# sharwarimarathe/GossipProtocol

Hardware: AMD Instinct MI355X
Metric: node-updates/sec (whole node) + achieved HBM GB/s %, imp3D push-sum 1e9 nodes (higher is better)
Workload: dtype f64; 1 GPU; push-sum rounds, Imp3D lattice, n=1000000000 (P=1000000000), steady state (all nodes active), seed 1; num_nodes=1000000000, population=1000000000, topology=Imp3D, algorithm=push-sum, parallelism=slab1, transport=none (one GPU), launcher=single process, activation_preroll_rounds=72

## Files before the change

gossipprotocol_amd/csrc/gp_host.hpp:

```cpp
#pragma once
#include <algorithm>
#include <array>
#include <chrono>
#include <cmath>
#include <cerrno>
#include <cstdarg>
#include <cstdio>
#include <cstdlib>
#include <cstring>
#include <optional>
#include <string>
#include <thread>
#include <vector>

#include <fcntl.h>
#include <sys/stat.h>
#include <unistd.h>

#include <rccl/rccl.h>

#include "../../include/gossip_hip.h"
#include "gp_internal.hpp"
#include "gp_full.hpp"
#include "gp_fullbin.hpp"

#include "gp_xchg.hpp"

using namespace gp;
#pragma GCC visibility push(hidden)

extern thread_local std::string g_err;
void set_err(const char* fmt, ...);
int check_device(int device);

#define HIP_TRY(expr)                                                                   \
    do {                                                                                \
        hipError_t e_ = (expr);                                                         \
        if (e_ != hipSuccess) {                                                         \
            set_err("%s failed: %s (%s:%d)", #expr, hipGetErrorString(e_), __FILE__, __LINE__); \
            return GP_EHIP;                                                             \
        }                                                                               \
    } while (0)

#define NCCL_TRY(expr)                                                                  \
    do {                                                                                \
        ncclResult_t r_ = (expr);                                                       \
        if (r_ != ncclSuccess) {                                                        \
            set_err("%s failed: %s (%s:%d)", #expr, ncclGetErrorString(r_), __FILE__, __LINE__); \
            return GP_ENCCL;                                                            \
        }                                                                               \
    } while (0)

constexpr int64_t BATCH = 1024;
static_assert(BATCH <= HIST, "alert ring must cover a batch");

struct ExpOverrides {
    KernelOverrides kernel;
    std::optional<uint32_t> fb_cap1, fb_cap2;
    std::optional<bool> fb_fused;
    std::optional<bool> rq8;
    std::optional<uint32_t> halo_cap;
    std::optional<uint32_t> xcap;
    std::optional<bool> no_pack;
    std::optional<uint32_t> ind4_wide;
    std::optional<bool> force_rccl;
    bool check_close = false;
};
ExpOverrides read_overrides();

struct Xfer { bool send; int peer; uint8_t* ptr; size_t bytes; };

struct Slab {
    DevState S{};
    int rank = 0;
    uint32_t hi = 0;
    uint32_t* pos = nullptr;
    uint8_t* xdst = nullptr;
    uint8_t* xsend = nullptr;
    uint8_t* xrecv = nullptr;
    uint32_t nedges = 0;
    XLayout xl;
    unsigned int* overflow = nullptr;
    bool lists = false;
    uint32_t nt = 0;
    uint32_t tb[XMAXH + 1] = {};
    uint32_t* gw = nullptr;
    uint16_t* xdr = nullptr;
    uint8_t* lwt = nullptr;
    uint32_t* xcnt = nullptr;
    uint8_t* xown = nullptr;
    bool bits = false;
    uint32_t* rbits_in = nullptr;
    uint32_t* tgt = nullptr;
    BitsLayout bl;
    double2* hsend[2] = {nullptr, nullptr};
    double2* hrecv[2] = {nullptr, nullptr};
    std::vector<Xfer> xhalo[2];
    std::vector<std::vector<Xfer>> xplan[2];
};

#pragma GCC visibility pop
struct gp_sim {
    gp_config cfg{};
    int device = 0;
    hipStream_t stream = nullptr;
    ExpOverrides exp;
    KernelPlan kplan;
    int grid = 1;
    int cus = 1;
    int64_t P = 0, T = 0, g = 0;
    int mode = MODE_SINGLE;
    int world = 1, rank = 0;
    std::vector<uint32_t> bounds;
    uint32_t halo = 0;
    std::vector<Slab> slab;
    ncclComm_t comm = nullptr;
    int64_t rounds_done = 0;
// ... 68 lines not shown
```

gossipprotocol_amd/csrc/gp_internal.hpp:

```cpp
#pragma once

#include <hip/hip_runtime.h>
#include <stdint.h>

#include <algorithm>
#include <cmath>
#include <vector>

#include "gp_block_plan.hpp"
#pragma GCC visibility push(hidden)
#include "gp_plan.hpp"
#include "gp_kernel_plan.hpp"
#pragma GCC visibility pop
#include "gp_device.hpp"

namespace gp {

constexpr int HIST = 4096;
constexpr uint32_t INJ_CHUNK = 65536;

constexpr int vmcnt_enc(int n) { return 0x0F70 | (n & 15) | ((n >> 4) << 14); }

template <typename T>
__device__ __forceinline__ T ld_const(const T* p) {
// ... 97 lines not shown
}

struct XHdr {
    unsigned long long mask;
    uint32_t base;
    uint32_t pad;
};
static_assert(sizeof(XHdr) == 16, "header words move as 16-byte loads");

struct DevState {
    Geom G;
    int topo, alg;
    uint32_t k0, k1;
    uint32_t seed_node;
    Ctl* ctl;
    double2* sw[2];
    uint8_t* nb[2];
    int32_t* c;
    uint32_t* rq[2];
    uint32_t rq8;
    uint32_t* rtg;
    uint32_t* sbits;
    uint64_t* rbits[2];
    uint32_t rbits_words;
    uint32_t* rnd;
    uint32_t* in_off;
    uint32_t* in_src;
    uint32_t* in_srcd;
    uint8_t* ind4;
    uint32_t* live_bits;
    uint32_t* chunk_live;
    uint32_t nchunks;
    int32_t* inc;
    uint32_t fb_s1, fb_nb1, fb_nb2, fb_cap1, fb_cap2;
    uint32_t fb_fused;
    uint32_t *fb_cnt1, *fb_cnt2;
    uint32_t *fb_hdr1, *fb_hdr2;
    double2 *fb_pay1, *fb_pay2;
    uint32_t lo, nloc, base;
    uint32_t ext_lo, ext_hi;
    uint32_t* rtag;
    double2* rmsg;
    uint32_t* rk;
    const XHdr* xhdr[2];
    const double2* xvals[2];
    uint32_t xnv;
    int kernel;
    uint32_t col_xsegs;
    uint32_t tile_walk;
    uint32_t tile_wx;
    uint32_t tile_stage_cap;
#ifdef GP_EXPERIMENTS
    uint32_t tile_no_full;
#endif
    uint32_t fuse_finalize;
    BlockPlan bplan;
    void* bface;
    void* bscratch;
    uint32_t tile_wide;
    uint32_t nedges;
    uint32_t* tq;
    uint32_t* wtiles;
    uint32_t rregions;
    uint32_t woff[RREG_MAX][9];
};
constexpr int TQ_STRIDE = 64;
hipError_t launch_round_tile_region(const DevState& S, uint32_t round, uint32_t h, int grid, hipStream_t st);

constexpr int TILE = 1024;
static_assert(XTILE == TILE, "the lists' tiles (gp_plan.hpp) are the tile kernels' tiles");

struct RoundArgs {
    const double2* swc;
    double2* swn;
    const uint8_t* nbc;
    uint8_t* nbn;
    const uint64_t* rbc;
    uint64_t* rbn;
    const uint32_t* in_off;
    const uint32_t* in_src;
    const uint32_t* in_srcd;
    const uint8_t* ind4;
    const uint32_t* rtag;
    const double2* rmsg;
    const uint32_t* rk;
    const XHdr* xhdr;
    const double2* xvals;
    uint32_t xnv;
    int32_t* c;
    Ctl* ctl;
    Geom G;
    uint32_t k0, k1, seed_node, ntiles;
    uint32_t lo, nloc, ext_lo, ext_hi;
    uint32_t walk;
    uint32_t wx;
    uint32_t stage_cap;
#ifdef GP_EXPERIMENTS
    uint32_t no_full;
#endif
    uint32_t fuse;
    const uint32_t* wt;
    uint32_t wo[9];
    uint32_t* tq;
    uint32_t* tq_next;
};

size_t block_face_bytes(const BlockPlan& p);
hipError_t block_kernel_setup(const BlockPlan& p);
bool block_plan_resident(const BlockPlan& p, int cus);
constexpr int BLOCK_EPOCH = 64;
constexpr size_t BLOCK_SCRATCH_BYTES = 4 * (144 + 12 * BLOCK_EPOCH);
hipError_t launch_round_block(const struct DevState& S, const BlockPlan& p, uint32_t r0, uint32_t nrounds, void* face,
                              void* scratch, hipStream_t st);

struct WaveArgs {
    const uint8_t* nbc;
    uint8_t* nbn;
    int32_t* c;
    uint32_t* rq_cur;
    uint32_t* rq_next;
    uint32_t rq8;
    const uint32_t* rnd;
    const uint32_t* rtg;
    uint32_t* sbits;
    Ctl* ctl;
    Geom G;
    uint32_t k0, k1, seed_node;
    uint32_t lo, nloc, base;
    uint32_t x_lo, x_hi, zsegs, yblocks, xs_len, nitems;
};

WaveArgs make_wave_args(const DevState& S, uint32_t round);

hipError_t launch_round_col(const WaveArgs& a, int topo, int alg, uint32_t round, int grid, hipStream_t st);
int col_blocks_per_cu(int topo, int alg);
hipError_t launch_col_seed_init(const DevState& S, hipStream_t st);

uint32_t rbits_words_for(uint32_t lo, uint32_t nloc);
RoundArgs make_round_args(const DevState& S, uint32_t round);
hipError_t launch_round_tile(const DevState& S, uint32_t round, int grid, hipStream_t st);
hipError_t launch_rbits_init(const DevState& S, int grid, hipStream_t st);
uint32_t ind4_bytes_for(uint32_t lo, uint32_t nloc);
hipError_t launch_pack_ind4(const DevState& S, uint32_t wide_at, int grid, hipStream_t st);
hipError_t launch_pack_src_deg(const uint32_t* src, uint32_t* out, uint32_t n, const Geom& G, int grid,
                               hipStream_t st);

hipError_t launch_ps_tile(const DevState& S, const RoundArgs& a, uint32_t round, int grid, hipStream_t st);
int ps_tile_resident_blocks(int topo, bool remote, int device);
hipError_t launch_gossip_tile(const DevState& S, const RoundArgs& a, uint32_t round, int grid, hipStream_t st);

namespace wide {
// ... 24 lines not shown
```

gossipprotocol_amd/csrc/gp_ps_tile.hip:

```cpp
#include <type_traits>

#include "gp_tile.hpp"

namespace gp {
#ifdef GP_TILE_WIDE
namespace wide {
#endif

constexpr int PRIO = 1;

namespace {

template <bool REMOTE>
struct PsSlots {
    static constexpr bool SNDPF = !REMOTE;
    static constexpr int SLOTS = SNDPF ? TILE + TILE / 8 : TILE + TILE / 8 + TILE / 16;
    static constexpr int FU = (SLOTS + TPB - 1) / TPB;
};

template <bool REMOTE>
struct TileLdsP {
    static constexpr int SLOTS = PsSlots<REMOTE>::SLOTS, SLOT_FU = PsSlots<REMOTE>::FU;
    uint32_t rows[W_ROWS + DMA_SLACK];
    uint32_t xm[W_PLANE + DMA_SLACK];
// ... 171 lines not shown
                    uint32_t hb[FU];
#pragma unroll
                    for (int m = 0; m < FU; ++m) {
                        const bool cand = pick[m] && isrc[m] - a.lo >= a.nloc;
                        const XHdr* hp = a.xhdr + (cand ? rkv[m] >> 6 : 0u);
                        hm[m] = *reinterpret_cast<const uint2*>(&hp->mask);
                        hb[m] = hp->base;
                    }
#pragma unroll
                    for (int m = 0; m < FU; ++m) asm volatile("" : "+v"(hm[m].x), "+v"(hm[m].y), "+v"(hb[m])::"memory");
#pragma unroll
                    for (int m = 0; m < FU; ++m) {
                        ridx[m] = 0u;
                        if (pick[m] && isrc[m] - a.lo >= a.nloc) {
                            const unsigned long long mk = ((unsigned long long)hm[m].y << 32) | hm[m].x;
                            const uint32_t bit = rkv[m] & 63u;
                            sent[m] = (mk >> bit) & 1ull;
                            ridx[m] = min(hb[m] + (uint32_t)__popcll(mk & ((1ull << bit) - 1ull)), a.xnv - 1u);
                        }
                    }
                }
                __builtin_amdgcn_s_setprio(PRIO);
#pragma unroll
                for (int m = 0; m < FU; ++m) {
                    const unsigned long long bal = __ballot(sent[m]);
                    if (lane == 0) L.bits[m * (TPB / 64) + wv] = bal;
                    if (sent[m]) {
                        const double2* src;
                        if constexpr (REMOTE) {
                            uint32_t xi = ridx[m];
                            asm volatile("" : "+v"(xi));
                            src = isrc[m] - a.lo >= a.nloc ? a.xvals + xi : swc + isrc[m];
                        } else {
                            src = swc + isrc[m];
                        }
                        __builtin_amdgcn_global_load_lds((gvoid_t*)src, (lvoid_t*)(L.msg + (m * TPB + wv * 64)), 16,
                                                         0, DMA_ONCE);
                    }
                }
                if (threadIdx.x == 0) {
                    unsigned long long z = 0ull;
                    asm volatile("" : "+v"(z));
                    L.bits[FU * (TPB / 64)] = z;
                }
            }
        }
        double2 own[NPT];
        const uint32_t b_rows = dma_stage_bytes(L.rows, a.nbc, (int64_t)j0 - H, (int64_t)j1 + H, a.ext_lo, a.ext_hi);
        uint32_t b_xm = 0, b_xp = 0;
        if (TOPO != LINE) {
            b_xm = dma_stage_bytes(L.xm, a.nbc, (int64_t)j0 - G.g2, (int64_t)j1 - G.g2, a.ext_lo, a.ext_hi);
            b_xp = dma_stage_bytes(L.xp, a.nbc, (int64_t)j0 + G.g2, (int64_t)j1 + G.g2, a.ext_lo, a.ext_hi);
        }
        if (lane < 2u * NPT) {
            uint32_t zl = lane;
            asm volatile("" : "+v"(zl));
            int64_t jn = (int64_t)T + (int64_t)((zl >> 1) * TPB + wv * 64u) + ((zl & 1u) ? 64 : -1);
            if (jn < (int64_t)a.ext_lo) jn = a.ext_lo;
            if (jn > (int64_t)a.ext_hi) jn = a.ext_hi;
            __builtin_amdgcn_global_load_lds((gvoid_t*)(swc + jn), (lvoid_t*)&L.zb[wv][0][0], 16, 0, 0);
        }
        if (TOPO == IMP3D) {
            const uint8_t* ip = a.ind4 + T / 2;
            asm volatile("" : "+s"(ip));
            dma_copy<DMA_ONCE>(L.ind, reinterpret_cast<const char*>(ip), TILE / 2);
        }
        if (dyn && threadIdx.x == 0) L.qn[it & 1] = claim;
        __builtin_amdgcn_s_setprio(0);
        __syncthreads();
        uint32_t cinc = 0;
        bool wide = false;
        if (TOPO == IMP3D) {
            const uint2 w2 = reinterpret_cast<const uint2*>(L.ind)[lane];
            auto nsum = [](uint32_t w) { return (((w & 0x0F0F0F0Fu) + ((w >> 4) & 0x0F0F0F0Fu)) * 0x01010101u) >> 24; };
            auto has15 = [](uint32_t w) { return (w & (w >> 1) & (w >> 2) & (w >> 3) & 0x11111111u) != 0u; };
            uint32_t incl = nsum(w2.x) + nsum(w2.y);
            wide = __ballot(has15(w2.x) || has15(w2.y)) != 0ull;
#pragma unroll
            for (int o = 1; o < 64; o <<= 1) {
                const uint32_t t = __shfl_up(incl, o, 64);
                if (lane >= (uint32_t)o) incl += t;
            }
            const uint32_t ex = __shfl_up(incl, 1, 64);
            cinc = lane == 0 ? 0u : ex;
        }
        uint32_t t_next = tw.t + tw.step;
        if (dyn) {
            t_next = __builtin_amdgcn_readfirstlane(L.qn[it & 1]);
            ++it;
            if (TOPO == IMP3D) {
                TileWalk nw = tw;
                nw.t = t_next;
                uint32_t nti;
                pf_tile = 0xFFFFFFFFu;
                if (nw.t < nw.end && nw.tile(nti)) {
                    const uint32_t nT = (a.lo / TILE + nti) * TILE;
                    pf_lo = ld_const(a.in_off + max(a.lo, nT));
                    pf_hi = ld_const(a.in_off + min(a.lo + a.nloc, nT + TILE));
                    pf_tile = nti;
                }
            }
        }

        bool full = j0 == T && j1 == T + TILE && (TOPO != IMP3D || (staged && !wide));
#ifdef GP_EXPERIMENTS
        if (a.no_full) full = false;
#endif
        auto tile_body = [&](auto full_c) {
        constexpr bool FULL = decltype(full_c)::value;
        uint32_t tid = threadIdx.x;
        asm volatile("" : "+v"(tid));
        const uint32_t lane = tid & 63u, wv = tid >> 6;
        uint32_t pend[(NPT + 1) / 2];
#pragma unroll
        for (int k = 0; k < (NPT + 1) / 2; ++k) pend[k] = 0u;
        {
            const uint32_t wbase = __builtin_amdgcn_readfirstlane(tid & ~63u);
            uint32_t wcx = 0, wcy = 0, wcz = 0;
            if (TOPO != LINE) {
                const uint32_t jw = T + wbase;
                wcx = fastdiv(jw, G.div_g2);
                const uint32_t rem = jw - wcx * G.g2;
                wcy = fastdiv(rem, G.div_g);
                wcz = rem - wcy * G.g;
            }
            constexpr uint32_t NDG = TOPO == LINE ? 0u : 4u;
            constexpr int NG = 1;
#pragma unroll
            for (int k0 = 0; k0 < NPT; k0 += NG) {
                __builtin_amdgcn_s_setprio(PRIO);
                uint32_t epre[NG], edeg[NG];
#pragma unroll
                for (int h = 0; h < NG; ++h) {
                    epre[h] = edeg[h] = 0u;
                    if (TOPO == IMP3D) {
                        const int k = k0 + h;
                        const uint32_t jl = k * TPB + tid;
                        const uint32_t d = (lds_byte(L.ind, jl >> 1) >> ((jl & 1u) * 4u)) & 15u;
                        uint32_t ex = mbcnt64(__ballot(d & 1u)) + 2u * mbcnt64(__ballot(d & 2u));
                        if (__ballot(d >= 4u)) ex += 4u * mbcnt64(__ballot(d & 4u)) + 8u * mbcnt64(__ballot(d & 8u));
                        const int wvu = __builtin_amdgcn_readfirstlane((int)wv);
                        epre[h] = (uint32_t)__builtin_amdgcn_readlane((int)cinc, 16 * k + 4 * wvu) + ex;
                        edeg[h] = d;
                    }
                }
                uint32_t gst[NG];
                double2 m[NG][NDG > 0 ? NDG : 1];
#pragma unroll
                for (int h = 0; h < NG; ++h) {
                    const int k = k0 + h;
                    const uint32_t j = T + k * TPB + tid;
                    if (TOPO != LINE && k > 0) {
                        wcz += TPB;
                        if (wcz >= G.g) {
                            const uint32_t q = fastdiv(wcz, G.div_g);
                            wcz -= q * G.g;
                            wcy += q;
                            if (wcy >= G.g) {
                                const uint32_t q2 = fastdiv(wcy, G.div_g);
                                wcy -= q2 * G.g;
                                wcx += q2;
                            }
                        }
                    }
                    const uint32_t jr = j - b_rows;
                    const uint32_t gbv = lds_byte(L.rows, jr);
                    uint32_t mask;
                    if (TOPO == LINE) {
                        mask = present_mask<TOPO>(j, G);
                    } else {
                        const uint32_t gm = G.g - 1u;
                        const bool interior = wcz >= 1u && wcz + 64u < gm && wcy >= 1u && wcy < gm && wcx >= 1u && wcx < gm;
                        mask = interior ? 63u : present_mask<TOPO>(j, G);
                    }
                    uint32_t from = 0;
                    if (TOPO == LINE) {
                        from |= ((mask & 1u) && (lds_byte(L.rows, (mask & 1u) ? jr - 1 : jr) & DIR_MASK) == 1u) ? 1u : 0u;
                        from |= ((mask & 2u) && (lds_byte(L.rows, (mask & 2u) ? jr + 1 : jr) & DIR_MASK) == 0u) ? 2u : 0u;
                    } else {
                        const uint32_t bxm = lds_byte(L.xm, (mask & 1u) ? j - G.g2 - b_xm : 0u);
                        const uint32_t bxp = lds_byte(L.xp, (mask & 2u) ? j + G.g2 - b_xp : 0u);
                        const uint32_t byp = lds_byte(L.rows, (mask & 4u) ? jr + G.g : jr);
                        const uint32_t bym = lds_byte(L.rows, (mask & 8u) ? jr - G.g : jr);
                        uint32_t bzp, bzm;
                        if constexpr (FULL) {
                            const uint32_t be = lds_byte(L.rows, lane == 63u ? jr + 1u : max(jr, 1u) - 1u);
                            bzp = (uint32_t)__builtin_amdgcn_mov_dpp((int)gbv, 0x130, 0xF, 0xF, true);
                            bzm = (uint32_t)__builtin_amdgcn_mov_dpp((int)gbv, 0x138, 0xF, 0xF, true);
                            if (lane == 63u) bzp = be;
                            if (lane == 0u) bzm = be;
                        } else {
                            bzp = lds_byte(L.rows, (mask & 16u) ? jr + 1 : jr);
                            bzm = lds_byte(L.rows, (mask & 32u) ? jr - 1 : jr);
                        }
                        from =((bxm & DIR_MASK) == 1u ? 1u : 0u) | ((bxp & DIR_MASK) == 0u ? 2u : 0u) |
                               ((byp & DIR_MASK) == 3u ? 4u : 0u) | ((bym & DIR_MASK) == 2u ? 8u : 0u) |
                               ((bzp & DIR_MASK) == 5u ? 16u : 0u) | ((bzm & DIR_MASK) == 4u ? 32u : 0u);
                        from &= mask;
                    }
                    if (!FULL && !(j >= j0 && j < j1)) from = 0u;
                    gst[h] = gbv | (mask << 8) | (from << 14) | (edeg[h] << 20);
                    own[k] = swc[FULL ? j : min(max(j, j0), j1 - 1u)];
#pragma unroll
                    for (uint32_t d = 0; d < NDG; ++d)
                        m[h][d] = ld_sw(swc + ((from >> d) & 1u ? nbr<TOPO>(j, d, G) : a.ext_hi));
                }
                __builtin_amdgcn_s_setprio(0);
#pragma unroll
                for (int h = 0; h < NG; ++h) {
                    const int k = k0 + h;
                    const uint32_t jl = k * TPB + tid;
                    const uint32_t j = T + jl;
                    const bool valid = FULL || (j >= j0 && j < j1);
                    uint32_t pwin = 0u, pqb = 0u;
                    if (TOPO == IMP3D && (FULL || (staged && !wide))) {
                        const uint32_t* bw = reinterpret_cast<const uint32_t*>(L.bits);
                        pqb = epre[h];
                        const uint32_t nd = gst[h] >> 20;
                        pwin = __builtin_amdgcn_alignbit(bw[(pqb >> 5) + 1], bw[pqb >> 5], pqb & 31u) & ((1u << nd) - 1u);
                    }
                    double2 zP = make_double2(0.0, 0.0), zM = zP;
                    {
                        constexpr uint32_t dP = TOPO == LINE ? 1u : 4u, dM = TOPO == LINE ? 0u : 5u;
                        const uint32_t from = (gst[h] >> 14) & 63u;
                        zP = dpp_double2<0x130>(own[k]);
                        zM = dpp_double2<0x138>(own[k]);
                        if (lane == 63u) zP = L.zb[wv][k][1];
                        if (lane == 0u) zM = L.zb[wv][k][0];
                        if (!((from >> dP) & 1u)) zP = make_double2(0.0, 0.0);
                        else if (!FULL && lane != 63u && j + 1u >= j1) zP = ld_sw(swc + j + 1);
                        if (!((from >> dM) & 1u)) zM = make_double2(0.0, 0.0);
                        else if (!FULL && lane != 0u && j <= j0) zM = ld_sw(swc + j - 1);
                    }
                    __builtin_amdgcn_s_waitcnt(vmcnt_enc(0));
                    if (valid) {
                        const uint32_t b = gst[h] & 0xFFu, mask = (gst[h] >> 8) & 63u, from = (gst[h] >> 14) & 63u;
                        const uint32_t deg = popc6(mask) + (TOPO == IMP3D ? 1u : 0u);
                        bool active = (b & B_ACTIVE) != 0;
                        const double2 sv = own[k];

                        const bool halve = active && deg > 0;
                        const double hf = halve ? 0.5 : 1.0;
                        double acc_s = sv.x * hf;
                        double acc_w = sv.y * hf;
                        auto fold = [&](const double2 mi) {
                            acc_s = __builtin_fma(mi.x, 0.5, acc_s);
                            acc_w = __builtin_fma(mi.y, 0.5, acc_w);
                        };
                        tiny |= (sv.y < 0x1p-1020) | (sv.x != 0.0 && sv.x < 0x1p-1020);
                        bool recv = from != 0;
                        if (TOPO == LINE) {
                            fold(zM);
                            fold(zP);
                        } else {
#pragma unroll
                            for (uint32_t d = 0; d < NDG; ++d) fold(m[h][d]);
                            fold(zP);
                            fold(zM);
                        }
                        if (TOPO == IMP3D) {
                            uint32_t e_b = e_lo + epre[h], e_e = e_b + (gst[h] >> 20);
                            if (!FULL && wide) {
                                e_b = a.in_off[j];
                                e_e = a.in_off[j + 1];
                            }
                            if (FULL || (staged && !wide)) {
                                uint32_t win = pwin;
                                while (win) {
                                    const uint32_t q = pqb + (uint32_t)__builtin_ctz(win);
                                    win &= win - 1u;
                                    fold(L.msg[q]);
                                    recv = true;
                                }
                            } else if (staged) {
                                const uint32_t* bw = reinterpret_cast<const uint32_t*>(L.bits);
                                const uint32_t qe = e_e - e_lo;
                                for (uint32_t q0 = e_b - e_lo; q0 < qe; q0 += 32u) {
                                    uint32_t win = __builtin_amdgcn_alignbit(bw[(q0 >> 5) + 1], bw[q0 >> 5], q0 & 31u);
                                    if (qe - q0 < 32u) win &= (1u << (qe - q0)) - 1u;
                                    while (win) {
                                        const uint32_t q = q0 + (uint32_t)__builtin_ctz(win);
                                        win &= win - 1u;
                                        fold(L.msg[q]);
                                        recv = true;
                                    }
                                }
                            } else {
                                for (uint32_t e = e_b; e < e_e; ++e) {
                                    const uint32_t i = in_src[e];
                                    bool sent;
                                    double2 mi = make_double2(0.0, 0.0);
                                    const bool rem = REMOTE && i - a.lo >= a.nloc;
                                    uint32_t xi = 0;
                                    if (rem) {
                                        const uint32_t k = a.rk[e];
                                        const XHdr h = a.xhdr[k >> 6];
                                        sent = (h.mask >> (k & 63u)) & 1ull;
                                        xi = min(h.base + (uint32_t)__popcll(h.mask & ((1ull << (k & 63u)) - 1ull)),
                                                 a.xnv - 1u);
                                    } else if (all_active) {
                                        const uint32_t di = popc6(present_mask<IMP3D>(i, G)) + 1u;
                                        sent = uniform(a.k0, a.k1, S_PUSHSUM, i, r, di) == di - 1u;
                                    } else {
                                        sent = (rbc[(i >> 6) - (a.lo >> 6)] >> (i & 63)) & 1ull;
                                    }
                                    if (sent) mi = rem ? a.xvals[xi] : ld_sw(swc + i);
                                    if (sent) {
                                        fold(mi);
                                        recv = true;
                                    }
                                }
                            }
                        }
                        uint32_t flags = b & (B_ACTIVE | B_CONV | (3u << CNT_SHIFT));
                        if (recv) {
                            if (!(b & B_CONV)) {
                                uint32_t cnt3 = (b >> CNT_SHIFT) & 3u;
                                cnt3 = ratio_moved(sv.x, sv.y, acc_s, acc_w) ? 0u : cnt3 + 1u;
                                flags = (flags & ~(3u << CNT_SHIFT)) | (cnt3 << CNT_SHIFT);
                                if (cnt3 == 3) {
                                    flags |= B_CONV;
                                    ++alerts;
                                }
                            }
                            if (!active) {
                                ++newly;
                                flags |= B_ACTIVE;
                                active = true;
                            }
                        }
                        pend[k >> 1] |= (mask | (active && deg > 0 ? 64u : 0u) | ((flags >> 3) << 7)) << (16 * (k & 1));
                        st_stream(swn + j, make_double2(acc_s, acc_w));
                    }
                }
                if (SNDPF && TOPO == IMP3D && k0 == 0) {
                    snd_tile = 0xFFFFFFFFu;
                    if (pf_tile != 0xFFFFFFFFu && pf_hi - pf_lo <= cap) {
                        snd_off = dma_stage_words(snd, srcp, pf_lo, pf_hi);
                        snd_tile = pf_tile;
                    }
                }
            }
        }
        {
            uint32_t node[NPT], x[NPT], y[NPT];
#pragma unroll
            for (int k = 0; k < NPT; ++k) node[k] = T + k * TPB + tid;
            philox2_batch<NPT>(node, r + 1, S_PUSHSUM, a.k0, a.k1, x, y);
#pragma unroll
            for (int k = 0; k < NPT; ++k) {
                const uint32_t jl = k * TPB + tid;
                const bool valid = FULL || (node[k] >= j0 && node[k] < j1);
                const uint32_t pk = pend[k >> 1] >> (16 * (k & 1));
                const uint32_t mask = pk & 63u;
                uint32_t dir = DIR_NONE;
                if (pk & 64u) dir = slot_to_dir_fast(mask, uniform_from(x[k], y[k], popc6(mask) + (TOPO == IMP3D ? 1u : 0u)));
                if (valid) reinterpret_cast<uint8_t*>(L.out)[jl] = (uint8_t)((((pk >> 7) & 15u) << 3) | dir);
                if (TOPO == IMP3D) {
                    const unsigned long long bits = __ballot(valid && dir == DIR_RANDOM);
                    if (lane == 0) {
                        const int64_t wi = (int64_t)((T + k * TPB + (tid & ~63u)) >> 6) - (int64_t)(a.lo >> 6);
                        if (wi >= 0) a.rbn[wi] = bits;
                    }
                }
            }
        }
        __syncthreads();
        for (uint32_t w = tid; w < (uint32_t)(TILE / 4); w += TPB) {
            const uint32_t jw = T + w * 4;
            if (FULL || (jw >= j0 && jw + 4 <= j1)) {
                st_stream(reinterpret_cast<uint32_t*>(a.nbn + T) + w, L.out[w]);
            } else {
                for (uint32_t b = 0; b < 4; ++b)
                    if (jw + b >= j0 && jw + b < j1) a.nbn[jw + b] = reinterpret_cast<const uint8_t*>(L.out)[w * 4 + b];
            }
        }
        };
        if (full) tile_body(std::true_type{});
        else tile_body(std::false_type{});
        tw.t = t_next;
    }
        if (!dyn || ++victim >= 8u) break;
        const uint32_t c = (blockIdx.x + victim) & 7u;
        tw.qc = a.tq + c * TQ_STRIDE;
        tw.wl = a.wt + a.wo[c];
        tw.end = a.wo[c + 1] - a.wo[c];
        if (threadIdx.x == 0) L.qn[it & 1] = atomicAdd(tw.qc, 1u);
        __syncthreads();
        tw.t = __builtin_amdgcn_readfirstlane(L.qn[it & 1]);
        ++it;
    }
}

__device__ __forceinline__ void block_counts(uint32_t (*red)[TPB / 64], uint32_t& x, uint32_t& y) {
    uint32_t tid = threadIdx.x;
    asm volatile("" : "+v"(tid));
    const uint32_t lane = tid & 63u, wv = tid >> 6;
#pragma unroll
    for (int o = 32; o > 0; o >>= 1) {
        x += __shfl_xor(x, o, 64);
        y += __shfl_xor(y, o, 64);
    }
    if (lane == 0) {
        red[0][wv] = x;
        red[1][wv] = y;
    }
    __syncthreads();
    if (threadIdx.x == 0) {
        x = 0;
        y = 0;
        for (int w = 0; w < TPB / 64; ++w) {
            x += red[0][w];
            y += red[1][w];
        }
    }
}

__device__ __forceinline__ void add_round_counts(Ctl* ctl, uint32_t x, uint32_t y) {
    unsigned long long d = 0;
    if (x) d += __hip_atomic_fetch_add(&ctl->round_alerts, (unsigned long long)x, __ATOMIC_RELAXED,
                                       __HIP_MEMORY_SCOPE_AGENT);
    if (y) d += __hip_atomic_fetch_add(&ctl->round_active, (unsigned long long)y, __ATOMIC_RELAXED,
                                       __HIP_MEMORY_SCOPE_AGENT);
    asm volatile("" ::"v"(d));
    __builtin_amdgcn_s_waitcnt(0);
}

template <int TOPO, bool REMOTE>
__global__ __launch_bounds__(TPB, GP_MINB) void k_ps_tile(RoundArgs a, uint32_t r) {
    __shared__ TileLdsP<REMOTE> L;
    __shared__ uint32_t snd[PsSlots<REMOTE>::SNDPF ? PsSlots<REMOTE>::SLOTS + DMA_SLACK : 1];
    Ctl* ctl = a.ctl;
// ... 66 lines not shown
```

gossipprotocol_amd/csrc/gp_setup.hip:

```cpp
#include "gp_host.hpp"

namespace {

inline const char* exp_env(const char* name) {
#ifdef GP_EXPERIMENTS
    return std::getenv(name);
#else
    (void)name;
    return nullptr;
#endif
}

}

ExpOverrides read_overrides() {
    auto count = [](const char* name, int least) -> std::optional<uint32_t> {
        const char* e = exp_env(name);
        if (!e) return std::nullopt;
        return (uint32_t)std::max(least, std::atoi(e));
    };
    auto number = [](const char* name) -> std::optional<int> {
        const char* e = exp_env(name);
        if (!e) return std::nullopt;
        return std::atoi(e);
    };
    auto is_one = [](const char* name) -> std::optional<bool> {
        const char* e = exp_env(name);
        if (!e) return std::nullopt;
        return e[0] == '1';
    };
    ExpOverrides o;
    KernelOverrides& k = o.kernel;
    if (const char* e = exp_env("GP_KERNEL"))
        k.kernel = !std::strcmp(e, "tile") ? KERNEL_TILE : !std::strcmp(e, "col") ? KERNEL_COL : !std::strcmp(e, "block") ? KERNEL_BLOCK : 0;
    k.xsegs = count("GP_XSEGS", 1);
    if (const auto v = number("GP_WALK")) k.walk = (uint32_t)*v;
    k.wx = count("GP_WX", 1);
    k.wide = is_one("GP_WIDE");
    k.rregions = number("GP_RREGIONS");
    k.xregions = number("GP_XREGIONS");
    if (const char* e = exp_env("GP_FUSE")) k.fuse = (uint32_t)(e[0] - '0');
    k.stage_cap = count("GP_STAGE_CAP", 0);
    k.no_full = is_one("GP_NO_FULLTILE");
    if (const char* e = exp_env("GP_GRID")) k.grid = e;
    o.fb_cap1 = count("GP_FB_CAP1", 1);
    o.fb_cap2 = count("GP_FB_CAP2", 1);
    o.fb_fused = is_one("GP_FB_FUSED");
    o.rq8 = is_one("GP_RQ8");
    o.halo_cap = count("GP_HALO_CAP", 1);
    o.xcap = count("GP_XCAP", 1);
    o.no_pack = is_one("GP_NO_PACK");
    o.ind4_wide = count("GP_IND4_WIDE", 1);
    o.force_rccl = is_one("GP_FORCE_RCCL");
    o.check_close = exp_env("GP_CHECK_CLOSE") != nullptr;
    return o;
}

namespace {

int make_bounds(gp_sim* s) {
    const int W = s->world;
    const int topo = s->cfg.topology;
    const SlabCut cut = topo == GP_FULL ? SlabCut::Full : topo == GP_LINE ? SlabCut::Line : SlabCut::Planes;
    switch (slab_bounds(s->P, s->g, W, cut, s->bounds, s->halo)) {
    case BoundsError::None:
        return GP_OK;
    case BoundsError::TooManyRanks:
        set_err("at most %d ranks are supported (got %d)", XMAXW, W);
        break;
    case BoundsError::FewerNodesThanRanks:
        if (topo == GP_FULL) set_err("full topology with %lld nodes cannot be split over %d ranks", (long long)s->P, W);
        else set_err("line with %lld nodes cannot be split over %d ranks", (long long)s->P, W);
        break;
    case BoundsError::FewerPlanesThanRanks:
        set_err("a %lld^3 lattice has fewer planes than ranks (%d)", (long long)s->g, W);
        break;
    }
    return GP_EINVAL;
}

int alloc_slab(gp_sim* s, Slab& sl, int r) {
    DevState& S = sl.S;
    const int W = s->world;
    sl.rank = r;
    const uint32_t lo = s->bounds[r], hi = s->bounds[r + 1];
    sl.hi = hi;
    S.topo = s->cfg.topology;
    S.alg = s->cfg.algorithm;
    S.G.P = (uint32_t)s->P;
    S.G.T = (uint32_t)s->T;
    S.G.g = (uint32_t)s->g;
    S.G.g2 = (uint32_t)(s->g * s->g);
    S.G.div_g = make_fastdiv(S.G.g ? S.G.g : 1);
    S.G.div_g2 = make_fastdiv(S.G.g2 ? S.G.g2 : 1);
    S.k0 = (uint32_t)s->cfg.seed;
    S.k1 = (uint32_t)(s->cfg.seed >> 32);
    S.seed_node = uniform(S.k0, S.k1, S_START, 0, 0, (uint32_t)s->T);
    S.lo = lo;
    S.nloc = hi - lo;
    S.ext_lo = r > 0 ? lo - s->halo : lo;
    S.ext_hi = r < W - 1 ? hi + s->halo : hi;
    S.base = S.ext_lo & ~3u;
    S.rtag = nullptr;
    S.rmsg = nullptr;
    S.rk = nullptr;
// ... 109 lines not shown
        int cus() const {
            hipDeviceProp_t prop;
            (void)hipGetDeviceProperties(&prop, s->device);
            return prop.multiProcessorCount;
        }
        bool block_resident(const BlockPlan& bp, int cus) const { return block_plan_resident(bp, cus); }
        int col_blocks_per_cu() const { return gp::col_blocks_per_cu(s->cfg.topology, s->cfg.algorithm); }
        int res4() const { return ps_tile_resident_blocks(r.tile_topo(), r.tile_remote(), s->device); }
        int res_wide() const { return wide::ps_tile_resident_blocks(r.tile_topo(), r.tile_remote(), s->device); }
    };
    const KernelFacts facts = gather_kernel_facts(shape, s->exp.kernel, Device{s, shape});
    KernelPlanError err;
    s->kplan = kernel_plan(shape, facts, s->exp.kernel, err);
    s->cus = std::max(1, facts.cus);
    s->grid = s->kplan.grid;
#ifdef GP_EXPERIMENTS
    if (err.bad_grid) {
        set_err("GP_GRID=%s: not a grid of 1..%d blocks", s->exp.kernel.grid->c_str(), err.grid_max);
        return GP_EINVAL;
    }
#endif
    return GP_OK;
}

int build_sim(gp_sim* s) {
    int rc;
    if ((rc = make_bounds(s))) return rc;
    if ((rc = plan_kernels(s))) return rc;
    const KernelPlan& kp = s->kplan;
    if (s->mode == MODE_VIRTUAL) {
        s->slab.resize(s->world);
        for (int w = 0; w < s->world; ++w) s->slab[w].rank = w;
    } else {
        s->slab.resize(1);
        s->slab[0].rank = s->rank;
    }
    for (Slab& sl : s->slab) {
        sl.S.kernel = kp.kernel;
        sl.S.tile_wide = kp.wide;
        sl.S.col_xsegs = kp.col_xsegs;
        sl.S.tile_walk = kp.walk;
        sl.S.tile_wx = kp.wx;
        sl.S.tile_stage_cap = kp.stage_cap;
        sl.S.fuse_finalize = kp.fuse_finalize;
        sl.S.bplan = kp.bplan;
        sl.S.bface = sl.S.bscratch = nullptr;
        if (kp.kernel == KERNEL_BLOCK) {
            if ((rc = dev_alloc(s, &sl.S.bface, block_face_bytes(kp.bplan))) || (rc = dev_alloc(s, &sl.S.bscratch, BLOCK_SCRATCH_BYTES)))
                return rc;
            HIP_TRY(block_kernel_setup(kp.bplan));
        }
#ifdef GP_EXPERIMENTS
        sl.S.tile_no_full = kp.no_full;
#endif
        if ((rc = alloc_slab(s, sl, sl.rank))) return rc;
        sl.S.rregions = kp.rregions;
        if (sl.S.tile_walk == 3) {
            std::vector<uint32_t> list;
            if (!build_walk_list(sl.S.lo, sl.S.nloc, sl.S.G.g2, sl.S.tile_wx, (int)sl.S.rregions, list, sl.S.woff)) {
                set_err("internal: walk-3 tile list does not cover the slab");
                return GP_EINVAL;
            }
            if ((rc = dev_alloc_t(s, &sl.S.wtiles, list.size() + 1))) return rc;
            HIP_TRY(hipMemcpy(sl.S.wtiles, list.data(), sizeof(uint32_t) * list.size(), hipMemcpyHostToDevice));
        }
    }
    if (s->cfg.topology == GP_IMP3D && (rc = build_imp3d(s))) return rc;
    if ((s->cfg.topology == GP_IMP3D || s->cfg.topology == GP_FULL) && s->world > 1 && (rc = setup_exchange(s)))
        return rc;
    if ((rc = setup_halo(s))) return rc;
    if (s->world > 1) build_transfers(s);
    if (hipHostMalloc((void**)&s->host_ctl, sizeof(Ctl), hipHostMallocDefault) != hipSuccess) {
        set_err("hipHostMalloc failed");
        return GP_ENOMEM;
    }
    Ctl& init = *s->host_ctl;
    std::memset(&init, 0, sizeof init);
    init.active_total = 1;
    init.all_active = s->P <= 1 ? 1u : 0u;
    init.inj_target = -1;
    init.inj_pick = -1;
    for (Slab& sl : s->slab) {
        DevState& S = sl.S;
        HIP_TRY(hipMemcpyAsync(S.ctl, &init, sizeof(Ctl), hipMemcpyHostToDevice, s->stream));
        HIP_TRY(launch_init(S, s->grid, s->stream));
        if (S.topo == IMP3D)
            HIP_TRY(col_gossip_counts(S) ? launch_col_seed_init(S, s->stream) : launch_rbits_init(S, s->grid, s->stream));
        if (S.alg == GOSSIP && S.topo != FULL) HIP_TRY(launch_injector_init(S, s->grid, s->stream));
    }
    if ((rc = exchange(s, 0))) return rc;
    if ((rc = finalize(s, 0, 0))) return rc;
    hipError_t e = hipStreamSynchronize(s->stream);
    if (e != hipSuccess) {
        set_err("initialisation failed: %s", hipGetErrorString(e));
        return GP_EHIP;
    }
    if (s->timing) {
        s->ev.resize((size_t)2 * BATCH * round_launches(s));
        for (auto& x : s->ev) HIP_TRY(hipEventCreate(&x));
    }
    return GP_OK;
}

}

int create_common(const gp_config* cfg, int mode, int world, int rank, const uint8_t* uid, gp_sim** out) {
// ... 51 lines not shown
```

gossipprotocol_amd/csrc/gp_tile_host.hip:

```cpp
#include <algorithm>

#include "gp_internal.hpp"

namespace gp {

constexpr int SETUP_TPB = 256;

__global__ __launch_bounds__(SETUP_TPB) void k_rbits_init(const uint8_t* nb, uint64_t* rb, uint32_t lo, uint32_t nloc,
                                                          uint32_t nwords) {
    const uint32_t j00 = lo & ~63u;
    for (uint32_t jb = blockIdx.x * SETUP_TPB; jb < nwords * 64u; jb += gridDim.x * SETUP_TPB) {
        const uint32_t j = j00 + jb + threadIdx.x;
        const bool bit = j >= lo && j - lo < nloc && (nb[j] & DIR_MASK) == DIR_RANDOM;
        const unsigned long long bits = __ballot(bit);
        if ((threadIdx.x & 63) == 0) rb[(j >> 6) - (lo >> 6)] = bits;
    }
}

uint32_t rbits_words_for(uint32_t lo, uint32_t nloc) { return tiles_for(lo, nloc) * (TILE / 64) + 16u; }

RoundArgs make_round_args(const DevState& S, uint32_t round) {
    const int cur = round & 1;
    RoundArgs a;
    a.swc = S.sw[cur] ? S.sw[cur] - S.base : nullptr;
    a.swn = S.sw[cur ^ 1] ? S.sw[cur ^ 1] - S.base : nullptr;
    a.nbc = S.nb[cur] ? S.nb[cur] - S.base : nullptr;
    a.nbn = S.nb[cur ^ 1] ? S.nb[cur ^ 1] - S.base : nullptr;
    a.rbc = S.rbits[cur];
    a.rbn = S.rbits[cur ^ 1];
    a.in_off = S.in_off ? S.in_off - S.lo : nullptr;
    a.in_src = S.in_src;
    a.in_srcd = S.in_srcd;
    a.ind4 = S.ind4 ? S.ind4 - (S.lo / TILE) * (TILE / 2) : nullptr;
    a.rtag = S.rtag;
    a.rmsg = S.rmsg;
    a.rk = S.rk;
    a.xhdr = S.xhdr[round & 1];
    a.xvals = S.xvals[round & 1];
    a.xnv = S.xnv;
    a.c = S.c ? S.c - S.lo : nullptr;
    a.lo = S.lo;
    a.nloc = S.nloc;
    a.ext_lo = S.ext_lo;
    a.ext_hi = S.ext_hi;
    a.ctl = S.ctl;
    a.G = S.G;
    a.k0 = S.k0;
    a.k1 = S.k1;
    a.seed_node = S.seed_node;
    a.ntiles = tiles_for(S.lo, S.nloc);
    a.walk = S.tile_walk;
    a.stage_cap = S.tile_stage_cap;
#ifdef GP_EXPERIMENTS
    a.no_full = S.tile_no_full;
#endif
    a.wx = S.tile_wx;
    a.fuse = S.fuse_finalize;
    a.wt = S.wtiles;
    for (int c = 0; c <= 8; ++c) a.wo[c] = S.woff[0][c];
    a.tq = S.tq + (round & 1) * 8 * TQ_STRIDE;
    a.tq_next = S.tq + ((round + 1) & 1) * 8 * TQ_STRIDE;
    return a;
}

hipError_t launch_round_tile(const DevState& S, uint32_t round, int grid, hipStream_t st) {
    if (S.rregions > 1) return hipErrorInvalidValue;
    const RoundArgs a = make_round_args(S, round);
    if (S.alg == PUSHSUM)
        return S.tile_wide ? wide::launch_ps_tile(S, a, round, grid, st) : launch_ps_tile(S, a, round, grid, st);
    if (S.tile_wide) return hipErrorInvalidValue;
    return launch_gossip_tile(S, a, round, grid, st);
}

__global__ __launch_bounds__(SETUP_TPB) void k_pack_src_deg(const uint32_t* src, uint32_t* out, uint32_t n, Geom G) {
    for (uint32_t e = blockIdx.x * SETUP_TPB + threadIdx.x; e < n; e += gridDim.x * SETUP_TPB) {
        const uint32_t i = src[e];
        const uint32_t deg = popc6(present_mask<IMP3D>(i, G)) + 1u;
        out[e] = i | ((deg - 4u) << 30);
    }
}

hipError_t launch_pack_src_deg(const uint32_t* src, uint32_t* out, uint32_t n, const Geom& G, int grid,
                               hipStream_t st) {
    hipLaunchKernelGGL(k_pack_src_deg, dim3(grid), dim3(SETUP_TPB), 0, st, src, out, n, G);
    return hipGetLastError();
}

__global__ __launch_bounds__(SETUP_TPB) void k_pack_ind4(const uint32_t* __restrict__ in_off, uint32_t lo, uint32_t nloc,
                                                         uint32_t j00, uint8_t* __restrict__ out, uint32_t nbytes,
                                                         uint32_t wide_at) {
    for (uint32_t b = blockIdx.x * SETUP_TPB + threadIdx.x; b < nbytes; b += gridDim.x * SETUP_TPB) {
        uint32_t v = 0;
#pragma unroll
        for (uint32_t h = 0; h < 2; ++h) {
            const uint32_t j = j00 + 2 * b + h;
            if (j - lo < nloc) {
                const uint32_t d = in_off[j + 1] - in_off[j];
                v |= (d >= wide_at ? 15u : d) << (4 * h);
            }
        }
        out[b] = (uint8_t)v;
    }
}

uint32_t ind4_bytes_for(uint32_t lo, uint32_t nloc) { return tiles_for(lo, nloc) * (TILE / 2) + 16u; }

hipError_t launch_pack_ind4(const DevState& S, uint32_t wide_at, int grid, hipStream_t st) {
// ... 14 lines not shown
```

Measured before the change: 84.04 billion node-updates/s.

## Shadow per-node random slot selection under neighbor load latency in push-sum tile

Adds a SHADOW variant of the push-sum tile body that computes each node's philox-based random target direction while its neighbor loads are in flight, instead of in a separate batched pass after the loop. It also computes the next node's gather decision one step ahead (software pipelining) and packs the finished direction directly into pend. Separately, the z-halo and ind4 DMA staging are reissued with block-wide thread indexing, and ind4 uses a single 16-byte LDS load per thread. The aim is to hide RNG ALU and decision work behind memory latency, at the cost of more live registers and scheduling barriers. Shadow mode is the default and can be disabled through an experiment flag.

Measured after the change: 85.67 billion node-updates/s (median of 6 runs). 1.02x the previous value.

```diff
diff --git a/gossipprotocol_amd/csrc/gp_host.hpp b/gossipprotocol_amd/csrc/gp_host.hpp
--- a/gossipprotocol_amd/csrc/gp_host.hpp
+++ b/gossipprotocol_amd/csrc/gp_host.hpp
@@ -63,6 +63,7 @@
     std::optional<uint32_t> xcap;
     std::optional<bool> no_pack;
     std::optional<uint32_t> ind4_wide;
+    std::optional<bool> slot_shadow;
     std::optional<bool> force_rccl;
     bool check_close = false;
 };
diff --git a/gossipprotocol_amd/csrc/gp_internal.hpp b/gossipprotocol_amd/csrc/gp_internal.hpp
--- a/gossipprotocol_amd/csrc/gp_internal.hpp
+++ b/gossipprotocol_amd/csrc/gp_internal.hpp
@@ -173,6 +173,7 @@
     uint32_t tile_stage_cap;
 #ifdef GP_EXPERIMENTS
     uint32_t tile_no_full;
+    uint32_t tile_slot_shadow;
 #endif
     uint32_t fuse_finalize;
     BlockPlan bplan;
@@ -218,6 +219,7 @@
     uint32_t stage_cap;
 #ifdef GP_EXPERIMENTS
     uint32_t no_full;
+    uint32_t slot_shadow;
 #endif
     uint32_t fuse;
     const uint32_t* wt;
diff --git a/gossipprotocol_amd/csrc/gp_ps_tile.hip b/gossipprotocol_amd/csrc/gp_ps_tile.hip
--- a/gossipprotocol_amd/csrc/gp_ps_tile.hip
+++ b/gossipprotocol_amd/csrc/gp_ps_tile.hip
@@ -247,18 +247,24 @@
             b_xm = dma_stage_bytes(L.xm, a.nbc, (int64_t)j0 - G.g2, (int64_t)j1 - G.g2, a.ext_lo, a.ext_hi);
             b_xp = dma_stage_bytes(L.xp, a.nbc, (int64_t)j0 + G.g2, (int64_t)j1 + G.g2, a.ext_lo, a.ext_hi);
         }
-        if (lane < 2u * NPT) {
-            uint32_t zl = lane;
-            asm volatile("" : "+v"(zl));
-            int64_t jn = (int64_t)T + (int64_t)((zl >> 1) * TPB + wv * 64u) + ((zl & 1u) ? 64 : -1);
-            if (jn < (int64_t)a.ext_lo) jn = a.ext_lo;
-            if (jn > (int64_t)a.ext_hi) jn = a.ext_hi;
-            __builtin_amdgcn_global_load_lds((gvoid_t*)(swc + jn), (lvoid_t*)&L.zb[wv][0][0], 16, 0, 0);
+        {
+            uint32_t zt = threadIdx.x;
+            asm volatile("" : "+v"(zt));
+            const uint32_t zl = zt & 63u, zw = zt >> 6;
+            if (zl < 2u * NPT) {
+                int64_t jn = (int64_t)T + (int64_t)((zl >> 1) * TPB + zw * 64u) + ((zl & 1u) ? 64 : -1);
+                if (jn < (int64_t)a.ext_lo) jn = a.ext_lo;
+                if (jn > (int64_t)a.ext_hi) jn = a.ext_hi;
+                __builtin_amdgcn_global_load_lds((gvoid_t*)(swc + jn), (lvoid_t*)&L.zb[zw][0][0], 16, 0, 0);
+            }
         }
         if (TOPO == IMP3D) {
             const uint8_t* ip = a.ind4 + T / 2;
             asm volatile("" : "+s"(ip));
-            dma_copy<DMA_ONCE>(L.ind, reinterpret_cast<const char*>(ip), TILE / 2);
+            uint32_t nt = threadIdx.x;
+            asm volatile("" : "+v"(nt));
+            if (nt < (uint32_t)(TILE / 32))
+                __builtin_amdgcn_global_load_lds((gvoid_t*)(ip + nt * 16u), (lvoid_t*)L.ind, 16, 0, DMA_ONCE);
         }
         if (dyn && threadIdx.x == 0) L.qn[it & 1] = claim;
         __builtin_amdgcn_s_setprio(0);
@@ -301,8 +307,9 @@
 #ifdef GP_EXPERIMENTS
         if (a.no_full) full = false;
 #endif
-        auto tile_body = [&](auto full_c) {
+        auto tile_body = [&](auto full_c, auto shadow_c) {
         constexpr bool FULL = decltype(full_c)::value;
+        constexpr bool SHADOW = decltype(shadow_c)::value;
         uint32_t tid = threadIdx.x;
         asm volatile("" : "+v"(tid));
         const uint32_t lane = tid & 63u, wv = tid >> 6;
@@ -320,104 +327,120 @@
                 wcz = rem - wcy * G.g;
             }
             constexpr uint32_t NDG = TOPO == LINE ? 0u : 4u;
-            constexpr int NG = 1;
-#pragma unroll
-            for (int k0 = 0; k0 < NPT; k0 += NG) {
+            auto decide = [&](const int k, uint32_t& gst, uint32_t& epre) {
+                epre = 0u;
+                uint32_t edeg = 0u;
+                if (TOPO == IMP3D) {
+                    const uint32_t jl = k * TPB + tid;
+                    const uint32_t d = (lds_byte(L.ind, jl >> 1) >> ((jl & 1u) * 4u)) & 15u;
+                    uint32_t ex = mbcnt64(__ballot(d & 1u)) + 2u * mbcnt64(__ballot(d & 2u));
+                    if (__ballot(d >= 4u)) ex += 4u * mbcnt64(__ballot(d & 4u)) + 8u * mbcnt64(__ballot(d & 8u));
+                    const int wvu = __builtin_amdgcn_readfirstlane((int)wv);
+                    epre = (uint32_t)__builtin_amdgcn_readlane((int)cinc, 16 * k + 4 * wvu) + ex;
+                    edeg = d;
+                }
+                const uint32_t j = T + k * TPB + tid;
+                if (TOPO != LINE && k > 0) {
+                    wcz += TPB;
+                    if (wcz >= G.g) {
+                        const uint32_t q = fastdiv(wcz, G.div_g);
+                        wcz -= q * G.g;
+                        wcy += q;
+                        if (wcy >= G.g) {
+                            const uint32_t q2 = fastdiv(wcy, G.div_g);
+                            wcy -= q2 * G.g;
+                            wcx += q2;
+                        }
+                    }
+                }
+                const uint32_t jr = j - b_rows;
+                const uint32_t gbv = lds_byte(L.rows, jr);
+                uint32_t mask;
+                if (TOPO == LINE) {
+                    mask = present_mask<TOPO>(j, G);
+                } else {
+                    const uint32_t gm = G.g - 1u;
+                    const bool interior = wcz >= 1u && wcz + 64u < gm && wcy >= 1u && wcy < gm && wcx >= 1u && wcx < gm;
+                    mask = interior ? 63u : present_mask<TOPO>(j, G);
+                }
+                uint32_t from = 0;
+                if (TOPO == LINE) {
+                    from |= ((mask & 1u) && (lds_byte(L.rows, (mask & 1u) ? jr - 1 : jr) & DIR_MASK) == 1u) ? 1u : 0u;
+                    from |= ((mask & 2u) && (lds_byte(L.rows, (mask & 2u) ? jr + 1 : jr) & DIR_MASK) == 0u) ? 2u : 0u;
+                } else {
+                    const uint32_t bxm = lds_byte(L.xm, (mask & 1u) ? j - G.g2 - b_xm : 0u);
+                    const uint32_t bxp = lds_byte(L.xp, (mask & 2u) ? j + G.g2 - b_xp : 0u);
+                    const uint32_t byp = lds_byte(L.rows, (mask & 4u) ? jr + G.g : jr);
+                    const uint32_t bym = lds_byte(L.rows, (mask & 8u) ? jr - G.g : jr);
+                    uint32_t bzp, bzm;
+                    if constexpr (FULL) {
+                        const uint32_t be = lds_byte(L.rows, lane == 63u ? jr + 1u : max(jr, 1u) - 1u);
+                        bzp = (uint32_t)__builtin_amdgcn_mov_dpp((int)gbv, 0x130, 0xF, 0xF, true);
+                        bzm = (uint32_t)__builtin_amdgcn_mov_dpp((int)gbv, 0x138, 0xF, 0xF, true);
+                        if (lane == 63u) bzp = be;
+                        if (lane == 0u) bzm = be;
+                    } else {
+                        bzp = lds_byte(L.rows, (mask & 16u) ? jr + 1 : jr);
+                        bzm = lds_byte(L.rows, (mask & 32u) ? jr - 1 : jr);
+                    }
+                    from =((bxm & DIR_MASK) == 1u ? 1u : 0u) | ((bxp & DIR_MASK) == 0u ? 2u : 0u) |
+                           ((byp & DIR_MASK) == 3u ? 4u : 0u) | ((bym & DIR_MASK) == 2u ? 8u : 0u) |
+                           ((bzp & DIR_MASK) == 5u ? 16u : 0u) | ((bzm & DIR_MASK) == 4u ? 32u : 0u);
+                    from &= mask;
+                }
+                if (!FULL && !(j >= j0 && j < j1)) from = 0u;
+                gst = gbv | (mask << 8) | (from << 14) | (edeg << 20);
+            };
+            constexpr bool AHEAD = SHADOW;
+            uint32_t gst_n = 0u, epre_n = 0u;
+            if (AHEAD) {
                 __builtin_amdgcn_s_setprio(PRIO);
-                uint32_t epre[NG], edeg[NG];
-#pragma unroll
-                for (int h = 0; h < NG; ++h) {
-                    epre[h] = edeg[h] = 0u;
-                    if (TOPO == IMP3D) {
-                        const int k = k0 + h;
-                        const uint32_t jl = k * TPB + tid;
-                        const uint32_t d = (lds_byte(L.ind, jl >> 1) >> ((jl & 1u) * 4u)) & 15u;
-                        uint32_t ex = mbcnt64(__ballot(d & 1u)) + 2u * mbcnt64(__ballot(d & 2u));
-                        if (__ballot(d >= 4u)) ex += 4u * mbcnt64(__ballot(d & 4u)) + 8u * mbcnt64(__ballot(d & 8u));
-                        const int wvu = __builtin_amdgcn_readfirstlane((int)wv);
-                        epre[h] = (uint32_t)__builtin_amdgcn_readlane((int)cinc, 16 * k + 4 * wvu) + ex;
-                        edeg[h] = d;
-                    }
-                }
-                uint32_t gst[NG];
-                double2 m[NG][NDG > 0 ? NDG : 1];
-#pragma unroll
-                for (int h = 0; h < NG; ++h) {
-                    const int k = k0 + h;
-                    const uint32_t j = T + k * TPB + tid;
-                    if (TOPO != LINE && k > 0) {
-                        wcz += TPB;
-                        if (wcz >= G.g) {
-                            const uint32_t q = fastdiv(wcz, G.div_g);
-                            wcz -= q * G.g;
-                            wcy += q;
-                            if (wcy >= G.g) {
-                                const uint32_t q2 = fastdiv(wcy, G.div_g);
-                                wcy -= q2 * G.g;
-                                wcx += q2;
-                            }
-                        }
-                    }
-                    const uint32_t jr = j - b_rows;
-                    const uint32_t gbv = lds_byte(L.rows, jr);
-                    uint32_t mask;
-                    if (TOPO == LINE) {
-                        mask = present_mask<TOPO>(j, G);
-                    } else {
-                        const uint32_t gm = G.g - 1u;
-                        const bool interior = wcz >= 1u && wcz + 64u < gm && wcy >= 1u && wcy < gm && wcx >= 1u && wcx < gm;
-                        mask = interior ? 63u : present_mask<TOPO>(j, G);
-                    }
-                    uint32_t from = 0;
-                    if (TOPO == LINE) {
-                        from |= ((mask & 1u) && (lds_byte(L.rows, (mask & 1u) ? jr - 1 : jr) & DIR_MASK) == 1u) ? 1u : 0u;
-                        from |= ((mask & 2u) && (lds_byte(L.rows, (mask & 2u) ? jr + 1 : jr) & DIR_MASK) == 0u) ? 2u : 0u;
-                    } else {
-                        const uint32_t bxm = lds_byte(L.xm, (mask & 1u) ? j - G.g2 - b_xm : 0u);
-                        const uint32_t bxp = lds_byte(L.xp, (mask & 2u) ? j + G.g2 - b_xp : 0u);
-                        const uint32_t byp = lds_byte(L.rows, (mask & 4u) ? jr + G.g : jr);
-                        const uint32_t bym = lds_byte(L.rows, (mask & 8u) ? jr - G.g : jr);
-                        uint32_t bzp, bzm;
-                        if constexpr (FULL) {
-                            const uint32_t be = lds_byte(L.rows, lane == 63u ? jr + 1u : max(jr, 1u) - 1u);
-                            bzp = (uint32_t)__builtin_amdgcn_mov_dpp((int)gbv, 0x130, 0xF, 0xF, true);
-                            bzm = (uint32_t)__builtin_amdgcn_mov_dpp((int)gbv, 0x138, 0xF, 0xF, true);
-                            if (lane == 63u) bzp = be;
-                            if (lane == 0u) bzm = be;
-                        } else {
-                            bzp = lds_byte(L.rows, (mask & 16u) ? jr + 1 : jr);
-                            bzm = lds_byte(L.rows, (mask & 32u) ? jr - 1 : jr);
-                        }
-                        from =((bxm & DIR_MASK) == 1u ? 1u : 0u) | ((bxp & DIR_MASK) == 0u ? 2u : 0u) |
-                               ((byp & DIR_MASK) == 3u ? 4u : 0u) | ((bym & DIR_MASK) == 2u ? 8u : 0u) |
-                               ((bzp & DIR_MASK) == 5u ? 16u : 0u) | ((bzm & DIR_MASK) == 4u ? 32u : 0u);
-                        from &= mask;
-                    }
-                    if (!FULL && !(j >= j0 && j < j1)) from = 0u;
-                    gst[h] = gbv | (mask << 8) | (from << 14) | (edeg[h] << 20);
+                decide(0, gst_n, epre_n);
+            }
+#pragma unroll
+            for (int k = 0; k < NPT; ++k) {
+                __builtin_amdgcn_s_setprio(PRIO);
+                uint32_t gst, epre;
+                if (AHEAD) {
+                    gst = gst_n;
+                    epre = epre_n;
+                } else {
+                    decide(k, gst, epre);
+                }
+                const uint32_t jl = k * TPB + tid;
+                const uint32_t j = T + jl;
+                double2 m[NDG > 0 ? NDG : 1];
+                {
+                    const uint32_t from = (gst >> 14) & 63u;
                     own[k] = swc[FULL ? j : min(max(j, j0), j1 - 1u)];
 #pragma unroll
                     for (uint32_t d = 0; d < NDG; ++d)
-                        m[h][d] = ld_sw(swc + ((from >> d) & 1u ? nbr<TOPO>(j, d, G) : a.ext_hi));
+                        m[d] = ld_sw(swc + ((from >> d) & 1u ? nbr<TOPO>(j, d, G) : a.ext_hi));
                 }
                 __builtin_amdgcn_s_setprio(0);
-#pragma unroll
-                for (int h = 0; h < NG; ++h) {
-                    const int k = k0 + h;
-                    const uint32_t jl = k * TPB + tid;
-                    const uint32_t j = T + jl;
+                if (SHADOW) __builtin_amdgcn_sched_barrier(0);
+                {
                     const bool valid = FULL || (j >= j0 && j < j1);
                     uint32_t pwin = 0u, pqb = 0u;
                     if (TOPO == IMP3D && (FULL || (staged && !wide))) {
                         const uint32_t* bw = reinterpret_cast<const uint32_t*>(L.bits);
-                        pqb = epre[h];
-                        const uint32_t nd = gst[h] >> 20;
+                        pqb = epre;
+                        const uint32_t nd = gst >> 20;
                         pwin = __builtin_amdgcn_alignbit(bw[(pqb >> 5) + 1], bw[pqb >> 5], pqb & 31u) & ((1u << nd) - 1u);
+                    }
+                    if (SHADOW) {
+                        uint32_t x, y;
+                        philox2(j, r + 1, S_PUSHSUM, a.k0, a.k1, x, y);
+                        const uint32_t mask = (gst >> 8) & 63u;
+                        const uint32_t cand = slot_to_dir_fast(mask, uniform_from(x, y, popc6(mask) + (TOPO == IMP3D ? 1u : 0u)));
+                        pend[k >> 1] |= cand << (16 * (k & 1));
+                        if (AHEAD && k + 1 < NPT) decide(k + 1, gst_n, epre_n);
+                        __builtin_amdgcn_sched_barrier(0);
                     }
                     double2 zP = make_double2(0.0, 0.0), zM = zP;
                     {
                         constexpr uint32_t dP = TOPO == LINE ? 1u : 4u, dM = TOPO == LINE ? 0u : 5u;
-                        const uint32_t from = (gst[h] >> 14) & 63u;
+                        const uint32_t from = (gst >> 14) & 63u;
                         zP = dpp_double2<0x130>(own[k]);
                         zM = dpp_double2<0x138>(own[k]);
                         if (lane == 63u) zP = L.zb[wv][k][1];
@@ -429,7 +452,7 @@
                     }
                     __builtin_amdgcn_s_waitcnt(vmcnt_enc(0));
                     if (valid) {
-                        const uint32_t b = gst[h] & 0xFFu, mask = (gst[h] >> 8) & 63u, from = (gst[h] >> 14) & 63u;
+                        const uint32_t b = gst & 0xFFu, mask = (gst >> 8) & 63u, from = (gst >> 14) & 63u;
                         const uint32_t deg = popc6(mask) + (TOPO == IMP3D ? 1u : 0u);
                         bool active = (b & B_ACTIVE) != 0;
                         const double2 sv = own[k];
@@ -449,12 +472,12 @@
                             fold(zP);
                         } else {
 #pragma unroll
-                            for (uint32_t d = 0; d < NDG; ++d) fold(m[h][d]);
+                            for (uint32_t d = 0; d < NDG; ++d) fold(m[d]);
                             fold(zP);
                             fold(zM);
                         }
                         if (TOPO == IMP3D) {
-                            uint32_t e_b = e_lo + epre[h], e_e = e_b + (gst[h] >> 20);
+                            uint32_t e_b = e_lo + epre, e_e = e_b + (gst >> 20);
                             if (!FULL && wide) {
                                 e_b = a.in_off[j];
                                 e_e = a.in_off[j + 1];
@@ -524,11 +547,15 @@
                                 active = true;
                             }
                         }
-                        pend[k >> 1] |= (mask | (active && deg > 0 ? 64u : 0u) | ((flags >> 3) << 7)) << (16 * (k & 1));
+                        if (SHADOW) {
+                            pend[k >> 1] |= ((active && deg > 0 ? 0u : (uint32_t)DIR_NONE) | (flags & 0x78u)) << (16 * (k & 1));
+                        } else {
+                            pend[k >> 1] |= (mask | (active && deg > 0 ? 64u : 0u) | ((flags >> 3) << 7)) << (16 * (k & 1));
+                        }
                         st_stream(swn + j, make_double2(acc_s, acc_w));
                     }
                 }
-                if (SNDPF && TOPO == IMP3D && k0 == 0) {
+                if (SNDPF && TOPO == IMP3D && k == 0) {
                     snd_tile = 0xFFFFFFFFu;
                     if (pf_tile != 0xFFFFFFFFu && pf_hi - pf_lo <= cap) {
                         snd_off = dma_stage_words(snd, srcp, pf_lo, pf_hi);
@@ -541,16 +568,23 @@
             uint32_t node[NPT], x[NPT], y[NPT];
 #pragma unroll
             for (int k = 0; k < NPT; ++k) node[k] = T + k * TPB + tid;
-            philox2_batch<NPT>(node, r + 1, S_PUSHSUM, a.k0, a.k1, x, y);
+            if (!SHADOW) philox2_batch<NPT>(node, r + 1, S_PUSHSUM, a.k0, a.k1, x, y);
 #pragma unroll
             for (int k = 0; k < NPT; ++k) {
                 const uint32_t jl = k * TPB + tid;
                 const bool valid = FULL || (node[k] >= j0 && node[k] < j1);
                 const uint32_t pk = pend[k >> 1] >> (16 * (k & 1));
-                const uint32_t mask = pk & 63u;
-                uint32_t dir = DIR_NONE;
-                if (pk & 64u) dir = slot_to_dir_fast(mask, uniform_from(x[k], y[k], popc6(mask) + (TOPO == IMP3D ? 1u : 0u)));
-                if (valid) reinterpret_cast<uint8_t*>(L.out)[jl] = (uint8_t)((((pk >> 7) & 15u) << 3) | dir);
+                uint32_t dir, nb;
+                if (SHADOW) {
+                    dir = pk & DIR_MASK;
+                    nb = pk & 0x7Fu;
+                } else {
+                    const uint32_t mask = pk & 63u;
+                    dir = DIR_NONE;
+                    if (pk & 64u) dir = slot_to_dir_fast(mask, uniform_from(x[k], y[k], popc6(mask) + (TOPO == IMP3D ? 1u : 0u)));
+                    nb = (((pk >> 7) & 15u) << 3) | dir;
+                }
+                if (valid) reinterpret_cast<uint8_t*>(L.out)[jl] = (uint8_t)nb;
                 if (TOPO == IMP3D) {
                     const unsigned long long bits = __ballot(valid && dir == DIR_RANDOM);
                     if (lane == 0) {
@@ -571,8 +605,14 @@
             }
         }
         };
-        if (full) tile_body(std::true_type{});
-        else tile_body(std::false_type{});
+#ifdef GP_EXPERIMENTS
+        if (!a.slot_shadow) {
+            if (full) tile_body(std::true_type{}, std::false_type{});
+            else tile_body(std::false_type{}, std::false_type{});
+        } else
+#endif
+        if (full) tile_body(std::true_type{}, std::true_type{});
+        else tile_body(std::false_type{}, std::true_type{});
         tw.t = t_next;
     }
         if (!dyn || ++victim >= 8u) break;
diff --git a/gossipprotocol_amd/csrc/gp_setup.hip b/gossipprotocol_amd/csrc/gp_setup.hip
--- a/gossipprotocol_amd/csrc/gp_setup.hip
+++ b/gossipprotocol_amd/csrc/gp_setup.hip
@@ -51,6 +51,7 @@
     o.xcap = count("GP_XCAP", 1);
     o.no_pack = is_one("GP_NO_PACK");
     o.ind4_wide = count("GP_IND4_WIDE", 1);
+    o.slot_shadow = is_one("GP_SLOT_SHADOW");
     o.force_rccl = is_one("GP_FORCE_RCCL");
     o.check_close = exp_env("GP_CHECK_CLOSE") != nullptr;
     return o;
@@ -266,6 +267,7 @@
         }
 #ifdef GP_EXPERIMENTS
         sl.S.tile_no_full = kp.no_full;
+        sl.S.tile_slot_shadow = s->exp.slot_shadow.value_or(true) ? 1u : 0u;
 #endif
         if ((rc = alloc_slab(s, sl, sl.rank))) return rc;
         sl.S.rregions = kp.rregions;
diff --git a/gossipprotocol_amd/csrc/gp_tile_host.hip b/gossipprotocol_amd/csrc/gp_tile_host.hip
--- a/gossipprotocol_amd/csrc/gp_tile_host.hip
+++ b/gossipprotocol_amd/csrc/gp_tile_host.hip
@@ -53,6 +53,7 @@
     a.stage_cap = S.tile_stage_cap;
 #ifdef GP_EXPERIMENTS
     a.no_full = S.tile_no_full;
+    a.slot_shadow = S.tile_slot_shadow;
 #endif
     a.wx = S.tile_wx;
     a.fuse = S.fuse_finalize;
```
